# TheSandvichMaker/BUAS-Pathtracer

Hardware: AMD Instinct MI355X
Metric: Mrays/s + samples/s/GPU at 1080p 256spp; 1/2/4/8-GPU scaling (higher is better)
Workload: dtype f32

## Files before the change

buas-pathtracer_amd/abi.py:

```python
import ctypes as C
import os

PKG_DIR = os.path.dirname(os.path.abspath(__file__))
LIB_PATH = os.path.join(PKG_DIR, "lib", "librt_mi355x.so")

RT_OK = 0
RT_ERROR_INVALID = 1
RT_ERROR_DEVICE = 2
RT_ERROR_OUT_OF_MEMORY = 3
RT_ERROR_CANCELLED = 4
RT_ERROR_NO_DEVICE = 5

RT_MATERIAL_MIRROR = 0x1
RT_MATERIAL_CHECKERS = 0x2
RT_MATERIAL_EMISSIVE = 0x4

RT_PRIMITIVE_NONE, RT_PRIMITIVE_PLANE, RT_PRIMITIVE_SPHERE, RT_PRIMITIVE_BOX, RT_PRIMITIVE_MESH = range(5)
RT_SAMPLING_UNIFORM, RT_SAMPLING_OPTIMIZED_BLUE_NOISE, RT_SAMPLING_STRATIFIED = range(3)
RT_SPLAT_STREAM, RT_SPLAT_EXACT, RT_SPLAT_ATOMIC = range(3)
RT_SHARD_TILES, RT_SHARD_PASSES = range(2)
RT_SHADOW_LAUNCH_AUTO, RT_SHADOW_LAUNCH_SEPARATE, RT_SHADOW_LAUNCH_MERGED = range(3)
(RT_INTEGRATOR_ADVANCED, RT_INTEGRATOR_WHITTED, RT_INTEGRATOR_GROUND_TRUTH_RECURSIVE,
 RT_INTEGRATOR_GROUND_TRUTH_ITERATIVE, RT_INTEGRATOR_NORMALS, RT_INTEGRATOR_DISTANCES) = range(6)
RT_INTEGRATOR_COUNT = 6
# ... 184 lines not shown
                ("max_leaf_size", C.c_uint32)]


P = C.POINTER

ABI_FUNCTIONS = {
    "rt_abi_version": (C.c_int, []),
    "rt_last_error": (C.c_char_p, []),
    "rt_device_count": (C.c_int, [P(C.c_int)]),
    "rt_integrator_name": (C.c_char_p, [C.c_int]),
    "rt_find_integrator": (C.c_int, [C.c_char_p]),
    "rt_integrator_supported": (C.c_int, [C.c_int]),
    "rt_scene_set_recursive_integrators": (C.c_int, [C.c_void_p, C.c_int]),
    "rt_scene_integrator_supported": (C.c_int, [C.c_void_p, C.c_int]),
    "rt_scene_set_ambient_light": (C.c_int, [C.c_void_p, P(V3)]),
    "rt_scene_upload": (C.c_int, [P(SceneDesc), C.c_int, P(C.c_void_p)]),
    "rt_scene_free": (C.c_int, [C.c_void_p]),
    "rt_render": (C.c_int, [C.c_void_p, P(Camera), P(Settings), P(FilterCache), P(TileSet), C.c_uint32,
                            P(AccumulationBuffer), P(Stats)]),
    "rt_render_device": (C.c_int, [C.c_void_p, P(Camera), P(Settings), P(FilterCache), P(TileSet), C.c_uint32,
                                   C.c_uint32, C.c_uint32, C.c_uint32, C.c_void_p, C.c_void_p, P(Stats)]),
    "rt_trace_samples": (C.c_int, [C.c_void_p, P(Camera), P(Settings), C.c_uint32, C.c_uint32, C.c_uint32,
                                   C.c_uint32, C.c_uint32, C.c_uint32, C.c_uint32, P(C.c_uint32), P(C.c_uint32),
                                   P(C.c_float), P(Stats)]),
    "rt_debug_intersect": (C.c_int, [C.c_void_p, C.c_uint32, P(RayQuery), C.c_int, P(HitRecord)]),
    "rt_debug_mesh_bvh4": (C.c_int, [P(BvhNode), C.c_uint32, P(C.c_float), C.c_uint32, P(C.c_uint32),
                                     P(C.c_uint32)]),
    "rt_debug_top_sequences": (C.c_int, [P(BvhNode), C.c_uint32, C.c_uint32, P(C.c_float), C.c_uint32,
                                         P(C.c_uint32)]),
    "rt_debug_claim_slots": (C.c_int, [P(C.c_uint32), C.c_uint32, C.c_uint32, C.c_uint32, P(C.c_uint32)]),
    "rt_debug_rank_slots": (C.c_int, [P(C.c_uint32), C.c_uint32, C.c_uint32, C.c_uint32, P(C.c_uint32)]),
    "rt_scene_ramp_stats": (C.c_int, [C.c_void_p, P(C.c_uint64), P(C.c_uint64)]),
    "rt_debug_verify_rcp": (C.c_int, [C.c_int, P(C.c_uint64), P(C.c_uint32)]),
    "rt_set_profiling": (C.c_int, [C.c_int]),
    "rt_set_profiling_stages": (C.c_int, [C.c_uint32]),
    "rt_set_path_pool": (C.c_int, [C.c_uint32]),
    "rt_set_splat_mode": (C.c_int, [C.c_int]),
    "rt_set_shard_mode": (C.c_int, [C.c_int]),
    "rt_set_env_sampling": (C.c_int, [C.c_int]),
    "rt_build_bvh": (C.c_int, [C.c_int, C.c_uint32, P(V3), P(V3), C.c_int, P(BvhNode), P(C.c_uint32), P(C.c_uint32)]),
    "rt_build_bvh_last_error": (C.c_char_p, []),
    "rt_render_picture": (C.c_int, [C.c_void_p, P(Camera), P(Settings), P(FilterCache), P(TileSet), C.c_uint32,
                                    C.c_uint32, C.c_uint32, P(PostSettings), P(C.c_uint32), P(Stats)]),
    "rt_cancel": (C.c_int, [C.c_void_p]),
    "rt_scene_default_config": (C.c_int, [P(SceneConfig)]),
    "rt_scene_get_config": (C.c_int, [C.c_void_p, P(SceneConfig)]),
    "rt_scene_set_config": (C.c_int, [C.c_void_p, P(SceneConfig)]),
    "rt_scene_stack_depth": (C.c_int, [C.c_void_p, P(C.c_uint32), P(C.c_uint32)]),
    "rt_postprocess_device": (C.c_int, [C.c_int, C.c_void_p, C.c_uint32, C.c_uint32, P(PostSettings), C.c_uint32,
                                        C.c_void_p, C.c_void_p]),
    "rt_postprocess": (C.c_int, [C.c_int, P(AccumulationBuffer), P(PostSettings), C.c_uint32, P(C.c_uint32)]),
    "rt_denoise_default_params": (C.c_int, [P(DenoiseParams)]),
    "rt_denoise_workspace_bytes": (C.c_size_t, [C.c_uint32, C.c_uint32]),
    "rt_denoise_device": (C.c_int, [C.c_int, C.c_void_p, C.c_void_p, C.c_void_p, C.c_uint32, C.c_uint32,
                                    P(DenoiseParams), C.c_void_p, C.c_void_p, C.c_void_p]),
    "rt_denoise": (C.c_int, [C.c_int, P(AccumulationBuffer), P(C.c_float), P(C.c_float), P(DenoiseParams),
                             P(C.c_float)]),
    "rt_render_picture_denoised": (C.c_int, [C.c_void_p, P(Camera), P(Settings), P(FilterCache), P(TileSet),
                                             C.c_uint32, C.c_uint32, C.c_uint32, P(PostSettings), P(DenoiseParams),
                                             C.c_uint32, P(C.c_uint32), P(Stats)]),
    "rt_render_feature_device": (C.c_int, [C.c_void_p, P(Camera), P(Settings), P(FilterCache), P(TileSet), C.c_uint32,
                                           C.c_uint32, C.c_uint32, C.c_uint32, C.c_int, C.c_void_p, C.c_void_p,
                                           P(Stats)]),
    "rt_render_feature": (C.c_int, [C.c_void_p, P(Camera), P(Settings), P(FilterCache), P(TileSet), C.c_uint32,
                                    C.c_int, P(AccumulationBuffer), P(Stats)]),
    "rt_render_features_device": (C.c_int, [C.c_void_p, P(Camera), P(Settings), P(FilterCache), P(TileSet), C.c_uint32,
# ... 121 lines not shown
```

buas-pathtracer_amd/csrc/rt_dmath.h:

```cpp
#pragma once
#include <hip/hip_runtime.h>
#include <stdint.h>
#include "../../include/rt_abi.h"

#ifdef RT_DMATH_HOST_TEST
#define RT_D inline
#else
#define RT_D __device__ __forceinline__
#endif

namespace rtd {

constexpr float PI_32 = 3.14159265359f;
constexpr float TAU_32 = 6.28318530717f;
constexpr float EPSILON = 0.001f;
constexpr float FLT_MAX_ = 3.402823466e+38F;

struct V3 { float x, y, z; };
struct V2 { float x, y; };

RT_D V3 v3(float x, float y, float z) { return {x, y, z}; }
RT_D V3 v3s(float s) { return {s, s, s}; }
RT_D V3 add(V3 a, V3 b) { return {a.x + b.x, a.y + b.y, a.z + b.z}; }
RT_D V3 sub(V3 a, V3 b) { return {a.x - b.x, a.y - b.y, a.z - b.z}; }
RT_D V3 mul(V3 a, V3 b) { return {a.x * b.x, a.y * b.y, a.z * b.z}; }
RT_D V3 divv(V3 a, V3 b) { return {a.x / b.x, a.y / b.y, a.z / b.z}; }
RT_D V3 muls(V3 a, float s) { return {a.x * s, a.y * s, a.z * s}; }
RT_D V3 smul(float s, V3 a) { return {s * a.x, s * a.y, s * a.z}; }
RT_D V3 divs(V3 a, float s) { return {a.x / s, a.y / s, a.z / s}; }
RT_D V3 sdiv(float s, V3 a) { return {s / a.x, s / a.y, s / a.z}; }
RT_D V3 neg(V3 a) { return {-a.x, -a.y, -a.z}; }
RT_D float rcp_cr(float x) {
#ifndef RT_DMATH_HOST_TEST
    const float a = __builtin_fabsf(x);
    if (a >= 0x1p-125f && a <= 0x1p125f) {
        const float r = __builtin_amdgcn_rcpf(x);
        return __builtin_fmaf(__builtin_fmaf(-x, r, 1.0f), r, r);
    }
#endif
    return 1.0f / x;
}
RT_D V3 rcp3(V3 a) { return {rcp_cr(a.x), rcp_cr(a.y), rcp_cr(a.z)}; }
RT_D float dot(V3 a, V3 b) { return a.x*b.x + a.y*b.y + a.z*b.z; }
RT_D V3 cross(V3 a, V3 b) { return {a.y*b.z - a.z*b.y, a.z*b.x - a.x*b.z, a.x*b.y - a.y*b.x}; }
RT_D float length_sq(V3 a) { return dot(a, a); }
RT_D float mn(float a, float b) { return a < b ? a : b; }
RT_D float mx(float a, float b) { return a > b ? a : b; }
RT_D float clampf_(float n, float a, float b) { return mx(a, mn(b, n)); }
RT_D float max3(V3 a) { return mx(a.x, mx(a.y, a.z)); }
RT_D V3 vabs(V3 a) { return {fabsf(a.x), fabsf(a.y), fabsf(a.z)}; }
RT_D V3 normalize(V3 a) { float r = rcp_cr(__builtin_sqrtf(dot(a, a))); return muls(a, r); }
RT_D V3 noz(V3 a) {
    V3 r = {0.0f, 0.0f, 0.0f};
    float lsq = length_sq(a);
    if ((lsq > 0.0001f) && (lsq < __builtin_inff())) r = divs(a, __builtin_sqrtf(lsq));
    return r;
}
RT_D float lerpf_(float a, float b, float t) { return a*(1.0f - t) + b*t; }
RT_D V3 lerp3(V3 a, V3 b, float t) { return add(muls(a, 1.0f - t), muls(b, t)); }
RT_D V3 reflect(V3 v, V3 n) { return sub(v, muls(n, 2.0f*dot(v, n))); }
RT_D float sign_of(float x) { return x < 0.0f ? -1.0f : 1.0f; }
RT_D float copy_sign(float v, float s) {
    return __uint_as_float((__float_as_uint(s) & 0x80000000u) | (__float_as_uint(v) & 0x7FFFFFFFu));
}
RT_D float comp(V3 a, int i) { return i == 0 ? a.x : (i == 1 ? a.y : a.z); }

struct M34 { float e[3][4]; };

RT_D V3 xform(const M34& a, V3 p, float pw) {
    return {p.x*a.e[0][0] + p.y*a.e[0][1] + p.z*a.e[0][2] + pw*a.e[0][3],
            p.x*a.e[1][0] + p.y*a.e[1][1] + p.z*a.e[1][2] + pw*a.e[1][3],
            p.x*a.e[2][0] + p.y*a.e[2][1] + p.z*a.e[2][2] + pw*a.e[2][3]};
}
RT_D V3 xform_normal(const M34& a, V3 n) {
    return {n.x*a.e[0][0] + n.y*a.e[0][1] + n.z*a.e[2][0],
// ... 195 lines not shown
```

buas-pathtracer_amd/csrc/rt_kernels.hip:

```cpp
#include <hip/hip_runtime.h>
#include <stdint.h>
#include <string.h>
#include <stdio.h>
#include <string>
#include <vector>
#include <chrono>
#include <algorithm>
#include <type_traits>
#include <cmath>
#include <mutex>
#include <cerrno>

#include "rt_dmath.h"

using namespace rtd;

#define HIP_OK(x) do { hipError_t e_ = (x); if (e_ != hipSuccess) { set_error(std::string(#x) + ": " + hipGetErrorString(e_)); return RT_ERROR_DEVICE; } } while (0)

namespace {
thread_local std::string g_error;
void set_error(const std::string& s) { g_error = s; }
uint32_t g_profiling = 0;
uint32_t g_pool_override = 0;
int g_splat_mode = RT_SPLAT_STREAM;
// ... 42 lines not shown
    uint32_t sky_w, sky_h;
    const float4* env_tab;
    uint32_t env_n, env_tx, env_tw, env_th;
    V3 top_sky, bot_sky;
    const uint8_t* strata;
    const uint8_t* bluenoise;
    const float4* blob;
    uint32_t blob_q;
    uint32_t off[7];
};
enum { BLOB_MATERIALS, BLOB_PRIMS, BLOB_PLANES, BLOB_INV, BLOB_FWD, BLOB_LIGHTS, BLOB_MESHES, BLOB_COUNT };
constexpr uint32_t LDS_SCENE_Q = 2048;
extern __shared__ float4 lds_scene[];

template <bool IN_LDS = false>
RT_D DevScene scene_in_lds(const DevScene& sc, float4* lds) {
    if (!IN_LDS && !sc.blob_q) return sc;
    for (uint32_t i = threadIdx.x; i < sc.blob_q; i += blockDim.x) lds[i] = sc.blob[i];
    __syncthreads();
    DevScene s = sc;
    const char* b = reinterpret_cast<const char*>(lds);
    s.materials = reinterpret_cast<const rt_material*>(b + sc.off[BLOB_MATERIALS]);
    s.prims = reinterpret_cast<const rt_primitive*>(b + sc.off[BLOB_PRIMS]);
    s.planes = reinterpret_cast<const rt_primitive*>(b + sc.off[BLOB_PLANES]);
    s.inv = reinterpret_cast<const M34*>(b + sc.off[BLOB_INV]);
    s.fwd = reinterpret_cast<const M34*>(b + sc.off[BLOB_FWD]);
    s.lights = reinterpret_cast<const uint32_t*>(b + sc.off[BLOB_LIGHTS]);
    s.meshes = reinterpret_cast<const DevMesh*>(b + sc.off[BLOB_MESHES]);
    return s;
}

struct Ray { V3 o, d, inv_d; uint32_t neg; float max_t; uint32_t zero; };

RT_D Ray make_ray(V3 o, V3 d, float far_clip) {
    Ray r;
    r.o = o; r.d = d;
    r.inv_d = rcp3(d);
    r.neg = (d.x < 0.0f ? 1u : 0u) | (d.y < 0.0f ? 2u : 0u) | (d.z < 0.0f ? 4u : 0u);
    r.zero = (d.x == 0.0f ? 1u : 0u) | (d.y == 0.0f ? 2u : 0u) | (d.z == 0.0f ? 4u : 0u);
    r.max_t = far_clip;
    return r;
}

RT_D bool ray_plane(const Ray& ray, V3 n, float d, float& t) {
    float denom = dot(n, ray.d);
    if (denom < -EPSILON) {
        float tt = (d - dot(n, ray.o)) / denom;
        if ((tt >= EPSILON) && (tt < t)) { t = tt; return true; }
    }
    return false;
}
RT_D bool ray_sphere(const Ray& ray, float r, float& t) {
    V3 o = ray.o;
    float rsq = r*r;
    float b = dot(ray.d, o);
    float c = dot(o, o) - rsq;
    float discr = (b*b - c);
    if (discr >= 0) {
        float root = __builtin_sqrtf(discr);
        float tn = -b - root;
        float tf = -b + root;
        float tt = (tn >= 0.0f ? tn : tf);
        if ((tt >= EPSILON) && (t > tt)) { t = tt; return true; }
    }
    return false;
}
RT_D bool ray_box(const Ray& ray, V3 br, float& t) {
    V3 m = ray.inv_d;
    V3 n = mul(m, ray.o);
    V3 k = mul(vabs(m), br);
    V3 t1 = sub(neg(n), k);
    V3 t2 = add(neg(n), k);
// ... 207 lines not shown
        return r;
    }
    const float4* seq = sc.top_seq;
    uint32_t list = 0, n = 0, next = 0;
    bool full = false;
    const uint32_t len = sc.top_seq_len;
    const bool plain = plain_ray(o, d);
    for (uint32_t i = 0; i < len; ++i) {
        const f32x8 e = ld_uniform_v<f32x8>(seq + 2*i);
        const float4 a = q4_of(e, 0), b = q4_of(e, 1);
        const uint32_t info = __float_as_uint(b.z), skip = __float_as_uint(b.w);
        bool pass = false;
        if (next == i) {
            float tn;
            pass = bv_static(wr, {a.x, a.y, a.z}, {a.w, b.x, b.y}, tn) && tn < r.t;
            next = pass ? ((info >> 31) ? skip : i + 1) : skip;
        }
        if (!(info >> 31) || __ballot(pass) == 0ull) continue;
        const uint32_t first = info & 0xFFFFFFu, end = first + ((info >> 24) & 127u);
        for (uint32_t j = first; j < end; ++j) {
            const float4* q = sc.leaf_rec + (size_t)j*LEAF_REC_Q;
            const f32x16 qa = ld_uniform_v<f32x16>(q);
            const float4 q3 = q4_of(qa, 3);
            const uint32_t pi = __float_as_uint(q3.x), tword = __float_as_uint(q3.y), type = tword & 0xFFu;
            if (!pass || pi == ignored) continue;
            const float4 q0 = q4_of(qa, 0), q1 = q4_of(qa, 1), q2 = q4_of(qa, 2);
            V3 io, id;
            object_ray(q0, q1, q2, tword & LEAF_TRANSLATE, plain, o, d, io, id);
            bool hit = false;
            if (type == RT_PRIMITIVE_SPHERE) {
                Ray ir; ir.o = io; ir.d = id;
                hit = ray_sphere(ir, q3.z, r.t);
            } else {
                const Ray ir = make_ray(io, id, 0.0f);
                if (type == RT_PRIMITIVE_MESH) {
                    const f32x8 qb = ld_uniform_v<f32x8>(q + 4);
                    const float4 q4 = q4_of(qb, 0), q5 = q4_of(qb, 1);
                    float tm;
                    n += 1u << 8;
                    if (bv_static(ir, {q4.y, q4.z, q4.w}, {q5.x, q5.y, q5.z}, tm) && tm < r.t) {
                        const uint32_t k = n & 0xFFu;
                        if (k < sc.mlist_max) list |= j << (6*k);
                        else full = true;
                        ++n;
                    }
                    continue;
                }
                if (type == RT_PRIMITIVE_BOX) hit = ray_box(ir, {q3.z, q3.w, ld_uniform(q + 4).x}, r.t);
            }
            if (hit) {
                r.code = pi;
                if (occ) { r.occluded = true; pass = false; next = 0xFFFFFFFFu; }
            }
        }
    }
    r.calls = n >> 8;
    if (r.occluded) return r;
    n &= 0xFFu;
    r.bvh = n > 0;
    r.mlist = full ? MLIST_FULL : (list | (n << 24));
    return r;
}

template <bool LST>
struct StepField {
    static constexpr uint32_t B = LST ? 8 : 6, M = (1u << B) - 1u;
    static constexpr uint32_t ENTRY = 1u, NODE = 1u << B, LEAF = 1u << 2*B, TRIS = 1u << 3*B,
// ... 127 lines not shown
    }

    template <bool SH>
    RT_D bool pop(const Stack& st, const rt_bvh_node* nodes, int base) {
        while (sp > base) {
            const uint2 e = st.template get<SH>(--sp);
            if (REF && e.x == REF_MARKER) {
                if (__uint_as_float(e.y) < t) { rp[0] += 2u; rp[1] += 1u; }
                continue;
            }
            if (__uint_as_float(e.y) < t) {
                unpack_node(nodes, e.x, cur_lf, cur_cnt, cur_ax);
                has_cur = true;
                return true;
            }
        }
        return false;
    }

    template <bool SH, bool FIN>
    RT_D void push_children4(const Stack& st, const float4* F, const float4* mid = nullptr) {
        const Ray r = cur_ray();
        const uint32_t meta = __float_as_uint(F[7].x), nb = cflags & 7u;
        const uint32_t g = (nb >> (meta & 3u)) & 1u;
        const uint32_t fa = (nb >> ((meta >> 2) & 3u)) & 1u;
        const uint32_t fb = (nb >> ((meta >> 4) & 3u)) & 1u;
        const uint32_t rec[4] = {__float_as_uint(F[6].x), __float_as_uint(F[6].y), __float_as_uint(F[6].z), __float_as_uint(F[6].w)};
        float tn[4];
        bool h[4];
        h[0] = bv_static<FIN>(r, {F[0].x, F[1].x, F[2].x}, {F[3].x, F[4].x, F[5].x}, tn[0]) && rec[0] != EMPTY4;
        h[1] = bv_static<FIN>(r, {F[0].y, F[1].y, F[2].y}, {F[3].y, F[4].y, F[5].y}, tn[1]) && rec[1] != EMPTY4;
        h[2] = bv_static<FIN>(r, {F[0].z, F[1].z, F[2].z}, {F[3].z, F[4].z, F[5].z}, tn[2]) && rec[2] != EMPTY4;
        h[3] = bv_static<FIN>(r, {F[0].w, F[1].w, F[2].w}, {F[3].w, F[4].w, F[5].w}, tn[3]) && rec[3] != EMPTY4;
        const uint32_t f1 = g ? fb : fa, f2 = g ? fa : fb;
        const uint32_t v[4] = {2u*g + f1, 2u*g + 1u - f1, 2u*(1u - g) + f2, 2u*(1u - g) + 1u - f2};
        bool far_marker = false;
        float far_tn = 0.0f;
        if (REF) {
            rp[0] += 2u; rp[1] += 1u;
            const V3 pc[2] = {{mid[0].x, mid[0].y, mid[0].z}, {mid[1].z, mid[1].w, mid[2].x}};
            const V3 rr[2] = {{mid[0].w, mid[1].x, mid[1].y}, {mid[2].y, mid[2].z, mid[2].w}};
#pragma unroll
            for (uint32_t c = 0; c < 2; ++c) {
                if ((c == 0 ? rec[1] : rec[3]) == EMPTY4) continue;
                float tc;
                const bool hc = bv_static<FIN>(r, pc[c], rr[c], tc);
                if (c == g) { if (hc && tc < t) { rp[0] += 2u; rp[1] += 1u; } }
                else if (hc) { far_marker = true; far_tn = tc; }
            }
        }
#pragma unroll
        for (int k = 3; k >= 0; --k) {
            const uint32_t i = v[k];
            const bool hi = i == 0 ? h[0] : i == 1 ? h[1] : i == 2 ? h[2] : h[3];
            const uint32_t ri = i == 0 ? rec[0] : i == 1 ? rec[1] : i == 2 ? rec[2] : rec[3];
            const float ti = i == 0 ? tn[0] : i == 1 ? tn[1] : i == 2 ? tn[2] : tn[3];
            if (hi) push<SH>(st, ri, ti);
            if (REF && k == 2 && far_marker) push<SH>(st, REF_MARKER, far_tn);
        }
    }

    static constexpr int PUSH_MAX = REF ? 5 : 4;
    using SF = StepField<LST>;
    uint32_t acc = 0;
    RT_D bool step(const DevScene& sc, const Stack& st) {
        if (__ballot(sp > SL - PUSH_MAX || !(cflags & 64u)) == 0ull) return step_impl<true, true>(sc, st);
// ... 1074 lines not shown
                }
                ro = add(I, smul(EPSILON, nd)); rd = nd;
                thr = mul(thr, lerp3(v3s(1.0f), rv3(mt.albedo), mt.metallic));
            } else if (mt.is_participating_medium) {
                if (inside) {
                    if (at > 0) --at;
                } else if (at < 63) {
                    ++at;
                    pool.mstack[(size_t)at*pool.n + slot] = (uint16_t)mt_id;
                }
                V3 fd = add(smul(eta, rd), muls(N, (eta*cos_i - cos_t)));
                ro = add(I, muls(fd, EPSILON)); rd = fd;
            } else {
                is_spec = 0;
                V3 albedo = evaluate_material(mt, I);
                V3 brdf = smul(1.0f / PI_32, albedo);
                if (st.next_event_estimation && (sc.light_count > 0 || ENV)) {
                    float lps = sample_1d(sc, ss, rng, S_LightSelection, bounce);
                    const float q = sc.light_count > 0 ? 0.5f : 1.0f;
                    const bool pick_env = ENV && lps < q;
                    if (ENV) lps = pick_env ? lps / q : (lps - q) / (1.0f - q);
                    float lrp = 0.0f;
                    uint32_t lid = pick_env ? 0u : pick_random_light(sc, st, lps, I, lrp);
                    if (ENV) lrp = lrp*(1.0f - q);
                    V2 s2 = sample_2d(sc, ss, rng, S_DirectLighting, bounce);
                    if (pick_env) {
                        V3 Lv = env_direction(sc, lps, s2);
                        float ndl = dot(N, Lv);
                        if (ndl > 0.0f) {
                            uint32_t tile;
                            V3 Le = sky_env(sc, Lv, tile);
                            float pe = env_pdf(sc, tile, Lv);
                            if (pe > 0.0f) {
                                float bpdf = (st.importance_sample_diffuse ? ndl / PI_32 : 1.0f / (2.0f*PI_32));
                                float pdf = st.use_mis ? q*pe + bpdf : q*pe;
                                sh_c = mul(mul(muls(thr, ndl / pdf), brdf), Le);
                                sh_o = add(I, muls(Lv, EPSILON));
                                sh_d = Lv;
                                sh_t = FLT_MAX_;
                                sh_light = 0;
                                cast_shadow = true;
                            }
                        }
                    } else {
                        const rt_primitive light = sc.prims[lid];
                        const M34 lf = load_m34(&sc.fwd[light.transform_index]);
                        V3 towards = normalize(sub(translation(lf), I));
                        if (light.type == RT_PRIMITIVE_SPHERE) {
                            float rad = light.p[0];
                            V3 Nl = map_to_hemisphere(neg(towards), s2);
                            V3 pw = xform(lf, muls(Nl, rad), 1.0f);
                            V3 Lv = sub(pw, I);
                            float dsq = length_sq(Lv);
                            float dist = __builtin_sqrtf(dsq);
                            Lv = divs(Lv, dist);
                            float A = 2.0f*PI_32*rad*rad;
                            float ndl = dot(N, Lv);
                            float nndl = -dot(Nl, Lv);
                            if (ndl > 0.0f && nndl > 0.0f) {
                                float sa = (nndl * A) / dsq;
                                float pdf;
                                if (st.use_mis) {
                                    float lpdf = rcp_cr(sa);
                                    float bpdf = (st.importance_sample_diffuse ? ndl / PI_32 : 1.0f / (2.0f*PI_32));
                                    pdf = lpdf + bpdf;
                                } else {
                                    pdf = rcp_cr(sa);
                                }
                                pdf *= lrp;
                                sh_c = mul(mul(muls(thr, dot(N, Lv) / pdf), brdf),
                                           rv3(sc.materials[light.material_id].emission_color));
                                sh_o = add(I, muls(Lv, EPSILON));
                                sh_d = Lv;
                                sh_t = dist - 2*EPSILON;
                                sh_light = lid;
                                cast_shadow = true;
                            }
                        }
                    }
                }
                V2 s2 = sample_2d(sc, ss, rng, S_IndirectLighting, bounce);
                V3 R;
                if (st.importance_sample_diffuse) {
                    R = map_to_cosine_weighted_hemisphere(N, s2);
                    thr = muls(thr, PI_32);
                } else {
                    R = map_to_hemisphere(N, s2);
                    thr = muls(thr, 2.0f*PI_32*dot(N, R));
                }
                thr = mul(thr, brdf);
                ro = add(I, muls(N, EPSILON)); rd = R;
            }
            if (st.russian_roulette && !is_spec) {
                float p = clampf_(max3(thr), 0.1f, 0.9f);
                float e = sample_1d(sc, ss, rng, S_Roulette, bounce);
                if (e > p) done = true;
                else thr = muls(thr, rcp_cr(p));
            }
        }
        if (!done) {
            if (st.importance_sample_diffuse) prev_pdf = dot(N, rd) / PI_32;
            ++bounce;
            if (bounce >= st.max_bounce_count) done = true;
        }
    } else {
        if (ENV) {
            uint32_t tile;
            V3 Le = sky_env(sc, rd, tile);
            if (!is_spec) {
                float wgt = 0.0f;
                if (st.use_mis) {
                    const float q = sc.light_count > 0 ? 0.5f : 1.0f;
                    float pe = env_pdf(sc, tile, rd);
                    float bpdf = (st.importance_sample_diffuse ? prev_pdf : 1.0f / (2.0f*PI_32));
                    float den = q*pe + bpdf;
                    wgt = den > 0.0f ? bpdf / den : 0.0f;
                }
                Le = smul(wgt, Le);
            }
            total = add(total, mul(thr, Le));
        } else {
            total = add(total, mul(thr, sample_sky(sc, rd)));
        }
        done = true;
    }
    return done;
}

template <int INTEG>
RT_D bool shade_bounce_gt(const DevScene& sc, const rt_settings& st, const Hit& h, V3& ro, V3& rd, V3& thr,
                          V3& total, uint32_t& bounce, Rng& rng) {
    constexpr bool FIRST_HIT = INTEG == RT_INTEGRATOR_NORMALS || INTEG == RT_INTEGRATOR_DISTANCES;
    if (h.code == RT_HIT_MISS) {
        if (FIRST_HIT) total = sample_sky(sc, rd);
// ... 647 lines not shown
                        ro = add(I, muls(nd, EPSILON)); rd = nd;
                    } else {
                        const V3 brdf = muls(evaluate_material(m, I), 1.0f / PI_32);
                        const V3 R = map_to_hemisphere(N, V2{r1, r2});
                        fs.put(level, 0, brdf, __uint_as_float(RF_DIFFUSE));
                        fs.put(level, 1, v3s(0.0f), mx(0.0f, dot(N, R)));
                        ro = add(I, muls(N, EPSILON)); rd = R;
                    }
                    ++level;
                }
            }
        }
        if (WHITTED) {
            V3 ill = {0, 0, 0};
            const uint32_t nlights = __ballot(lit) ? sc.light_count : 0u;
            for (uint32_t li = 0; li < nlights; ++li) {
                bool cast_shadow = false;
                V3 sh_o = {0, 0, 0}, sh_d = {0, 0, 0}, sh_c = {0, 0, 0};
                float sh_t = 0.0f;
                uint32_t sh_light = 0;
                if (lit) {
                    const uint32_t lid = sc.lights[li];
                    const rt_primitive light = sc.prims[lid];
                    const V2 s2 = sample_2d(sc, ss, rng, S_DirectLighting, 0);
                    if (light.type == RT_PRIMITIVE_SPHERE) {
                        const M34 lf = load_m34(&sc.fwd[light.transform_index]);
                        const V3 towards = normalize(sub(translation(lf), I));
                        const float rad = light.p[0];
                        const V3 Nl = map_to_hemisphere(neg(towards), s2);
                        const V3 pw = xform(lf, muls(Nl, rad), 1.0f);
                        V3 Lv = sub(pw, I);
                        const float dsq = length_sq(Lv);
                        const float dist = __builtin_sqrtf(dsq);
                        Lv = divs(Lv, dist);
                        const float A = 2.0f*PI_32*rad*rad;
                        const float ndl = dot(N, Lv);
                        const float nndl = -dot(Nl, Lv);
                        if (ndl > 0.0f && nndl > 0.0f) {
                            sh_o = add(I, muls(Lv, EPSILON));
                            sh_d = Lv;
                            sh_t = dist - 2*EPSILON;
                            sh_light = lid;
                            sh_c = divs(smul(nndl*A*ndl, rv3(sc.materials[light.material_id].emission_color)), dsq);
                            cast_shadow = true;
                        }
                    }
                }
                Prologue spro = {};
                if (cast_shadow) spro = ray_prologue(sc, sh_o, sh_d, sh_t, true, sh_light);
                n_calls[1] += cast_shadow ? spro.calls : 0u;
                Traversal<true, LST, STACK_LDS, REF> tr;
                bool tracing = cast_shadow && !spro.occluded && spro.bvh;
                n_traced_sh += tracing ? 1u : 0u;
                if (tracing) {
                    tr.init_rec(sc, stk, sh_o, sh_d, spro.inv_d, sh_t, sh_light, spro.mlist);
                    tracing = tr.mode != TM_DONE;
                }
                for (int k = 1; __ballot(tracing); ++k) {
                    if (tracing && !tr.step(sc, stk)) tracing = false;
                    if (k % StepField<LST>::H == 0) tally[1].flush(tr.acc);
                }
                tally[1].flush(tr.acc);
                if (REF) tally[1].flush_ref(tr.rc);
                if (cast_shadow && !spro.occluded && (!spro.bvh || !tr.occluded)) ill = add(ill, sh_c);
                n_shadow += cast_shadow ? 1u : 0u;
            }
            if (lit) {
// ... 493 lines not shown
RT_D float post_clamp(float n, float a, float b) { return mx(a, mn(b, n)); }
RT_D float sigmoidal_contrast(float x, float contrast, float midpoint) {
    float curve;
    if (x < midpoint) {
        float scale = (1.0f / midpoint)*x;
        curve = midpoint*(scale*scale);
    } else {
        float y = (1.0f / (1.0f - midpoint));
        float scale = y - y*x;
        curve = 1.0f - (1.0f - midpoint)*(scale*scale);
    }
    return lerpf_(x, curve, contrast);
}
RT_D float remap_tpdf(float x) {
    float orig = 2.0f*x - 1.0f;
    x = orig*(1.0f / __builtin_sqrtf(fabsf(orig)));
    x = mx(-1.0f, x);
    x = x - sign_of(x);
    return x;
}
__global__ void __launch_bounds__(256) k_verify_rcp(uint32_t base, unsigned long long* out) {
    const uint32_t t = blockIdx.x*256 + threadIdx.x, stride = gridDim.x*256;
    for (uint32_t i = 0; i < 16; ++i) {
        const uint32_t bits = base + t + i*stride;
        const float x = __uint_as_float(bits);
        const float a = rcp_cr(x), b = 1.0f / x;
        if (__float_as_uint(a) != __float_as_uint(b) && !(a != a && b != b)) {
            atomicAdd(out, 1ull);
            atomicMin(out + 1, (unsigned long long)bits);
        }
    }
}

__global__ void __launch_bounds__(256) k_post(const float4* px, uint32_t w, uint32_t h, rt_post_settings post,
                                              const uint8_t* noise, uint32_t* out) {
    const uint32_t x = blockIdx.x*64 + (threadIdx.x & 63), y = blockIdx.y*4 + (threadIdx.x >> 6);
    if (x >= w || y >= h) return;
    const size_t i = (size_t)y*w + x;
    const float4 s = px[i];
    V3 c = {0.0f, 0.0f, 0.0f};
    if ((s.x != s.x) || (s.y != s.y) || (s.z != s.z) || (s.w != s.w)) {
        c = {0.0f, 255.0f, 255.0f};
    } else if (s.w > 0.001f) {
        c = {s.x / s.w, s.y / s.w, s.z / s.w};
        c = {mx(c.x, 0.0f), mx(c.y, 0.0f), mx(c.z, 0.0f)};
        if (post.exposure != 0.0f) c = smul(d_powf(2.0f, post.exposure), c);
        if (post.tonemapping) c = {1.0f - d_expf(-c.x), 1.0f - d_expf(-c.y), 1.0f - d_expf(-c.z)};
        if (post.srgb_transform) {
            const float g = 1.0f / 2.23333f;
            c = {d_powf(c.x, g), d_powf(c.y, g), d_powf(c.z, g)};
        }
        if (post.contrast != 0.0f)
            c = {sigmoidal_contrast(c.x, post.contrast, post.midpoint), sigmoidal_contrast(c.y, post.contrast, post.midpoint),
                 sigmoidal_contrast(c.z, post.contrast, post.midpoint)};
        c = smul(255.0f, c);
        const uint8_t* d = noise + 3*((size_t)(y & 255u)*256 + (x & 255u));
        c.x = c.x + (0.5f + remap_tpdf((1.0f / 255.0f)*(float)d[0]));
        c.y = c.y + (0.5f + remap_tpdf((1.0f / 255.0f)*(float)d[1]));
        c.z = c.z + (0.5f + remap_tpdf((1.0f / 255.0f)*(float)d[2]));
    } else if (s.w < -0.01f) {
        c = {-255.0f*s.w, 0.0f, -255.0f*s.w};
    }
    const uint32_t r = (uint8_t)post_clamp(c.x, 0.0f, 255.0f);
    const uint32_t g = (uint8_t)post_clamp(c.y, 0.0f, 255.0f);
    const uint32_t b = (uint8_t)post_clamp(c.z, 0.0f, 255.0f);
    out[i] = (255u << 24) | (r << 16) | (g << 8) | b;
// ... 1201 lines not shown
        auto within = [](const rt_bvh_node* n, size_t count) {
            for (size_t i = 0; i < count; ++i) {
                const float c[3] = {n[i].bv_p.x, n[i].bv_p.y, n[i].bv_p.z}, r[3] = {n[i].bv_r.x, n[i].bv_r.y, n[i].bv_r.z};
                for (int k = 0; k < 3; ++k)
                    if (!(std::fabs(c[k]) + std::fabs(r[k]) <= 1099511627776.0f)) return false;
            }
            return true;
        };
        ds.finite_boxes = (within(d->bvh_nodes, d->bvh_node_count) && within(mnodes.data(), mnodes.size())) ? 1u : 0u;
    }
    if (top_depth + mesh_depth + 2 > STACK_DEPTH) {
        char msg[224];
        snprintf(msg, sizeof(msg), "rt_scene_upload: BVH too deep for the device's BVH4 traversal stack: needs %u entries "
                 "(top level %u + mesh BVH4 %u + 2), %d available (the device's bound, not the reference's BVH2 stack)",
                 top_depth + mesh_depth + 2, top_depth, mesh_depth, STACK_DEPTH);
        set_error(msg);
        return fail(RT_ERROR_INVALID);
    }
    s->bvh_depth = top_depth + mesh_depth;
    s->bvh_depth_ref = top_depth + std::max(mesh_depth, mesh_depth_ref);
    if (s->cfg.traversal_ref && s->bvh_depth_ref + 2 > STACK_DEPTH) {
        set_error("rt_scene_upload: traversal_ref needs more than the 64-entry traversal stack for this BVH");
        return fail(RT_ERROR_INVALID);
    }
    {
        auto u2f = [](uint32_t u) { float f; memcpy(&f, &u, 4); return f; };
        std::vector<float4> rec((size_t)d->bvh_index_count*LEAF_REC_Q, make_float4(0, 0, 0, 0));
        for (uint32_t j = 0; j < d->bvh_index_count; ++j) {
            const uint32_t pi = d->bvh_indices[j];
            const rt_primitive& p = d->primitives[pi];
            float4* q = rec.data() + (size_t)j*LEAF_REC_Q;
            const M34& iv = inv[p.transform_index];
            for (int r = 0; r < 3; ++r) q[r] = make_float4(iv.e[r][0], iv.e[r][1], iv.e[r][2], iv.e[r][3]);
            if (p.type == RT_PRIMITIVE_MESH) {
                const rt_mesh& M = d->meshes[p.mesh_index];
                rt_bvh_node rn = {};
                if (M.node_count) rn = M.nodes[0];
                const uint32_t root = root4[p.mesh_index];
                q[3] = make_float4(u2f(pi), u2f(p.type), u2f(meshes[p.mesh_index].node_offset), u2f(meshes[p.mesh_index].tri_offset));
                q[4] = make_float4(u2f(root), rn.bv_p.x, rn.bv_p.y, rn.bv_p.z);
                if (M.node_count) q[5] = make_float4(rn.bv_r.x, rn.bv_r.y, rn.bv_r.z, 1.0f);
                else q[5] = make_float4(-1.0f, -1.0f, -1.0f, 0.0f);
            } else {
                bool translate = std::isfinite(iv.e[0][3]) && std::isfinite(iv.e[1][3]) && std::isfinite(iv.e[2][3]);
                for (int r = 0; r < 3; ++r)
                    for (int c = 0; c < 3; ++c) translate = translate && iv.e[r][c] == (r == c ? 1.0f : 0.0f);
                q[3] = make_float4(u2f(pi), u2f(p.type | (translate ? LEAF_TRANSLATE : 0u)), p.p[0], p.p[1]);
                q[4] = make_float4(p.p[2], 0.0f, 0.0f, 0.0f);
            }
        }
        rec.resize(rec.size() + FETCH_Q, make_float4(0, 0, 0, 0));
        if ((err = upload(s, rec.data(), rec.size(), &ds.leaf_rec))) return fail(err);
    }
    if ((err = upload(s, meshes.data(), meshes.size(), &ds.meshes))) return fail(err);
    tris.resize(tris.size() + FETCH_Q, make_float4(0, 0, 0, 0));
    if ((err = upload(s, tris.data(), tris.size(), &ds.tris))) return fail(err);
    if ((err = upload(s, orig.data(), orig.size(), &ds.tri_orig))) return fail(err);
    if ((err = upload(s, normals.data(), normals.size(), &ds.normals))) return fail(err);
    mnodes.resize(mnodes.size() + (FETCH_Q*16 + 31)/32, rt_bvh_node{});
    if ((err = upload(s, mnodes.data(), mnodes.size(), &ds.mnodes_src))) return fail(err);
    {
        std::vector<rt_bvh_node> tl(mnodes.size());
        for (uint32_t m = 0; m < d->mesh_count; ++m) {
            const uint32_t off = meshes[m].node_offset, n = d->meshes[m].node_count;
            std::vector<rt_bvh_node> one = traversal_layout(mnodes.data() + off, n);
            std::copy(one.begin(), one.end(), tl.begin() + off);
        }
        if ((err = upload(s, tl.data(), tl.size(), &ds.mnodes))) return fail(err);
    }
    ds.mnodes4 = nullptr;
    {
        const uint32_t n4 = (uint32_t)(mnodes4.size() / 8);
        bool bad = false;
        for (uint32_t m = 0; m < d->mesh_count; ++m)
            bad |= root4[m] < (1u << 28) && root4[m] >= n4 && d->meshes[m].node_count && !d->meshes[m].nodes[0].count;
        for (size_t k = 0; k < n4 && !bad; ++k)
            for (int j = 0; j < 4; ++j) {
                uint32_t r;
                memcpy(&r, &(&mnodes4[8*k + 6].x)[j], 4);
                bad |= r != EMPTY4 && r < (1u << 28) && r >= n4;
// ... 777 lines not shown
    return RT_OK;
}

int rt_debug_top_sequences(const rt_bvh_node* nodes, uint32_t node_count, uint32_t index_count,
                           float* out, uint32_t out_cap_entries, uint32_t* out_len) {
    if (!nodes || !out_len) { set_error("null argument"); return RT_ERROR_INVALID; }
    uint32_t len = 0;
    std::vector<float4> q = top_sequences(nodes, node_count, index_count, len);
    *out_len = len;
    if (q.empty()) { set_error("top level too large for the prologue"); return RT_ERROR_INVALID; }
    if (out && out_cap_entries >= 8*len) memcpy(out, q.data(), q.size()*sizeof(float4));
    return (out && out_cap_entries < 8*len) ? RT_ERROR_INVALID : RT_OK;
}

int rt_debug_verify_rcp(int device, uint64_t* out_mismatches, uint32_t* out_first_bits) {
    if (!out_mismatches || !out_first_bits) { set_error("null argument"); return RT_ERROR_INVALID; }
    int err = bind_device(device);
    if (err) return err;
    unsigned long long* d = nullptr;
    HIP_OK(hipMalloc(&d, 2*sizeof(unsigned long long)));
    const unsigned long long init[2] = {0ull, 0xFFFFFFFFull};
    HIP_OK(hipMemcpy(d, init, sizeof(init), hipMemcpyHostToDevice));
    for (uint32_t chunk = 0; chunk < 16; ++chunk)
        k_verify_rcp<<<(1u << 28) / (256*16), 256>>>(chunk << 28, d);
    HIP_OK(hipGetLastError());
    unsigned long long h[2];
    HIP_OK(hipMemcpy(h, d, sizeof(h), hipMemcpyDeviceToHost));
    (void)hipFree(d);
    *out_mismatches = h[0];
    *out_first_bits = (uint32_t)h[1];
    return RT_OK;
}

int rt_debug_intersect(rt_scene* s, uint32_t count, const rt_ray_query* rays, int occlusion, rt_hit_record* out) {
    if (!s || !rays || !out) { set_error("null argument"); return RT_ERROR_INVALID; }
    if (!count) return RT_OK;
    HIP_OK(hipSetDevice(s->device));
    rt_ray_query* d_r = nullptr; rt_hit_record* d_o = nullptr;
    HIP_OK(hipMalloc(&d_r, sizeof(rt_ray_query)*count));
    HIP_OK(hipMalloc(&d_o, sizeof(rt_hit_record)*count));
    HIP_OK(hipMemcpy(d_r, rays, sizeof(rt_ray_query)*count, hipMemcpyHostToDevice));
    uint2* d_sp = nullptr;
    const uint32_t dgrid = (count + 127) / 128;
    HIP_OK(hipMalloc(&d_sp, sizeof(uint2)*(size_t)(STACK_DEPTH - STACK_LDS)*dgrid*128));
    if (occlusion) k_debug_intersect<true><<<dgrid, 128>>>(s->ds, d_r, d_o, count, d_sp);
    else k_debug_intersect<false><<<dgrid, 128>>>(s->ds, d_r, d_o, count, d_sp);
    HIP_OK(hipGetLastError());
    HIP_OK(hipDeviceSynchronize());
    (void)hipFree(d_sp);
    HIP_OK(hipMemcpy(out, d_o, sizeof(rt_hit_record)*count, hipMemcpyDeviceToHost));
    (void)hipFree(d_r); (void)hipFree(d_o);
    return RT_OK;
}

}

#include "rt_internal.h"
void rt_internal_set_error(const char* message) { set_error(message); }
int rt_internal_bind_device(int device) { return bind_device(device); }
int rt_internal_scene_device(const rt_scene* scene) { return scene->device; }
int rt_internal_scene_cancelled(const rt_scene* scene) { return scene->cancel; }
```

include/rt_abi.h:

```cpp
#ifndef RT_ABI_H
#define RT_ABI_H

#include <stdint.h>
#include <stddef.h>

#ifdef __cplusplus
extern "C" {
#endif

#define RT_ABI_VERSION 8

enum rt_status {
    RT_OK                 = 0,
    RT_ERROR_INVALID      = 1,
    RT_ERROR_DEVICE       = 2,
    RT_ERROR_OUT_OF_MEMORY= 3,
    RT_ERROR_CANCELLED    = 4,
    RT_ERROR_NO_DEVICE    = 5,
};

typedef struct rt_v3 { float x, y, z; } rt_v3;
typedef struct rt_m4x4 { float e[4][4]; } rt_m4x4;
typedef struct rt_m4x4inv { rt_m4x4 forward, inverse; } rt_m4x4inv;

// ... 211 lines not shown
              const rt_filter_cache* filter, const rt_tile_set* tiles,
              uint32_t total_frame_index, rt_accumulation_buffer* accum, rt_stats* stats);

int rt_render_device(rt_scene* scene, const rt_camera* camera, const rt_settings* settings,
                     const rt_filter_cache* filter, const rt_tile_set* tiles,
                     uint32_t total_frame_index, uint32_t w, uint32_t h, uint32_t frame_count,
                     float* d_pixels, void* hip_stream, rt_stats* stats);

int rt_render_picture(rt_scene* scene, const rt_camera* camera, const rt_settings* settings,
                      const rt_filter_cache* filter, const rt_tile_set* tiles, uint32_t total_frame_index,
                      uint32_t w, uint32_t h, const rt_post_settings* post, uint32_t* out_bgra, rt_stats* stats);

int rt_trace_samples(rt_scene* scene, const rt_camera* camera, const rt_settings* settings,
                     uint32_t w, uint32_t h, uint32_t tile_w, uint32_t tile_h,
                     uint32_t frame_count, uint32_t total_frame_index,
                     uint32_t count, const uint32_t* pixel_xy, const uint32_t* sample_offset,
                     float* out_rgbjj, rt_stats* stats);

int rt_debug_intersect(rt_scene* scene, uint32_t count, const rt_ray_query* rays,
                       int occlusion, rt_hit_record* out);

int rt_debug_mesh_bvh4(const rt_bvh_node* nodes, uint32_t node_count, float* out, uint32_t out_cap_nodes,
                       uint32_t* out_nodes, uint32_t* out_root_record);
int rt_debug_top_sequences(const rt_bvh_node* nodes, uint32_t node_count, uint32_t index_count,
                           float* out, uint32_t out_cap_entries, uint32_t* out_len);

int rt_debug_claim_slots(const uint32_t* free_w, uint32_t nwaves, uint32_t first_claim, uint32_t count,
                         uint32_t* out_slots);
int rt_debug_rank_slots(const uint32_t* free_w, uint32_t nwaves, uint32_t first_rank, uint32_t count,
                        uint32_t* out_slots);
int rt_scene_ramp_stats(const rt_scene* scene, uint64_t* out_iterations, uint64_t* out_paths);

int rt_debug_verify_rcp(int device, uint64_t* out_mismatches, uint32_t* out_first_bits);

int rt_postprocess_device(int device, const float* d_pixels, uint32_t w, uint32_t h,
                          const rt_post_settings* post, uint32_t total_frame_index,
                          uint32_t* d_bgra, void* hip_stream);

int rt_postprocess(int device, const rt_accumulation_buffer* accum, const rt_post_settings* post,
                   uint32_t total_frame_index, uint32_t* out_bgra);

typedef struct rt_denoise_params {
    int32_t iterations;
    float   sigma_color;
    float   sigma_guide[2];
    float   firefly_clamp;
    int32_t reserved[3];
} rt_denoise_params;
int    rt_denoise_default_params(rt_denoise_params* out);
size_t rt_denoise_workspace_bytes(uint32_t w, uint32_t h);
int rt_denoise_device(int device, const float* d_beauty, const float* d_guide0, const float* d_guide1,
                      uint32_t w, uint32_t h, const rt_denoise_params* p, void* d_workspace,
                      float* d_out, void* hip_stream);
int rt_denoise(int device, const rt_accumulation_buffer* beauty, const float* guide0, const float* guide1,
               const rt_denoise_params* p, float* out_pixels);
int rt_render_picture_denoised(rt_scene* scene, const rt_camera* camera, const rt_settings* settings,
                               const rt_filter_cache* filter, const rt_tile_set* tiles, uint32_t total_frame_index,
                               uint32_t w, uint32_t h, const rt_post_settings* post, const rt_denoise_params* p,
                               uint32_t guide_spp, uint32_t* out_bgra, rt_stats* stats);

enum rt_feature { RT_FEATURE_NORMAL = 0, RT_FEATURE_DISTANCE = 1, RT_FEATURE_ALBEDO = 2, RT_FEATURE_COUNT = 3 };
int rt_render_feature_device(rt_scene* scene, const rt_camera* camera, const rt_settings* settings,
                             const rt_filter_cache* filter, const rt_tile_set* tiles, uint32_t total_frame_index,
                             uint32_t w, uint32_t h, uint32_t frame_count, int feature, float* d_pixels,
                             void* hip_stream, rt_stats* stats);
int rt_render_feature(rt_scene* scene, const rt_camera* camera, const rt_settings* settings,
// ... 165 lines not shown
```

Baseline: 14400.

## Replace IEEE divides with exact reciprocal-FMA sequences and reuse world inv_d for translated instances

Replaces divisions by PI and by the light distance with reciprocal-multiply plus FMA correction sequences meant to give bit-identical results, and adds device verification entry points for both. Mesh instances whose transform is a pure translation now carry the LEAF_TRANSLATE flag, so when a whole wave qualifies the world ray's inverse direction is reused instead of recomputing three reciprocals. The BVH4 child push in the non-reference path is rewritten as branch-free slot arithmetic. These trim ALU work in shading and traversal, at the cost of extra range checks and code size.

Result: faster. 14780 (median of 6 runs) (+2.6%).

```diff
diff --git a/buas-pathtracer_amd/abi.py b/buas-pathtracer_amd/abi.py
--- a/buas-pathtracer_amd/abi.py
+++ b/buas-pathtracer_amd/abi.py
@@ -240,6 +240,8 @@
     "rt_debug_rank_slots": (C.c_int, [P(C.c_uint32), C.c_uint32, C.c_uint32, C.c_uint32, P(C.c_uint32)]),
     "rt_scene_ramp_stats": (C.c_int, [C.c_void_p, P(C.c_uint64), P(C.c_uint64)]),
     "rt_debug_verify_rcp": (C.c_int, [C.c_int, P(C.c_uint64), P(C.c_uint32)]),
+    "rt_debug_verify_div_pi": (C.c_int, [C.c_int, P(C.c_uint64), P(C.c_uint32)]),
+    "rt_debug_verify_div3": (C.c_int, [C.c_int, C.c_uint32, P(C.c_float), P(C.c_uint64), P(C.c_uint32)]),
     "rt_set_profiling": (C.c_int, [C.c_int]),
     "rt_set_profiling_stages": (C.c_int, [C.c_uint32]),
     "rt_set_path_pool": (C.c_int, [C.c_uint32]),
diff --git a/buas-pathtracer_amd/csrc/rt_dmath.h b/buas-pathtracer_amd/csrc/rt_dmath.h
--- a/buas-pathtracer_amd/csrc/rt_dmath.h
+++ b/buas-pathtracer_amd/csrc/rt_dmath.h
@@ -41,6 +41,36 @@
     return 1.0f / x;
 }
 RT_D V3 rcp3(V3 a) { return {rcp_cr(a.x), rcp_cr(a.y), rcp_cr(a.z)}; }
+struct ByPi {
+    static constexpr float D = PI_32, C = 0x1.45f306p-2f;
+};
+static_assert(ByPi::C == 1.0f / ByPi::D, "ByPi::C is the rounded reciprocal of PI_32");
+template <class K>
+RT_D float div_const(float x) {
+    const float a = __builtin_fabsf(x);
+    if (a >= 0x1p-100f && a <= FLT_MAX_) {
+        const float q0 = x * K::C;
+        return __builtin_fmaf(__builtin_fmaf(-K::D, q0, x), K::C, q0);
+    }
+    return x / K::D;
+}
+RT_D float div_pi(float x) { return div_const<ByPi>(x); }
+constexpr float DIV3_LO = 0x1p-46f, DIV3_HI = 0x1p46f;
+RT_D bool div3_in_range(float x) { const float a = __builtin_fabsf(x); return a >= DIV3_LO && a <= DIV3_HI; }
+RT_D V3 div3_by(V3 n, float d) {
+#ifndef RT_DMATH_HOST_TEST
+    if (div3_in_range(d) && div3_in_range(n.x) && div3_in_range(n.y) && div3_in_range(n.z)) {
+        const float r0 = __builtin_amdgcn_rcpf(d);
+        const float r = __builtin_fmaf(__builtin_fmaf(-d, r0, 1.0f), r0, r0);
+        V3 q = {n.x * r, n.y * r, n.z * r};
+        q = {__builtin_fmaf(__builtin_fmaf(-d, q.x, n.x), r, q.x), __builtin_fmaf(__builtin_fmaf(-d, q.y, n.y), r, q.y),
+             __builtin_fmaf(__builtin_fmaf(-d, q.z, n.z), r, q.z)};
+        return {__builtin_fmaf(__builtin_fmaf(-d, q.x, n.x), r, q.x), __builtin_fmaf(__builtin_fmaf(-d, q.y, n.y), r, q.y),
+                __builtin_fmaf(__builtin_fmaf(-d, q.z, n.z), r, q.z)};
+    }
+#endif
+    return {n.x / d, n.y / d, n.z / d};
+}
 RT_D float dot(V3 a, V3 b) { return a.x*b.x + a.y*b.y + a.z*b.z; }
 RT_D V3 cross(V3 a, V3 b) { return {a.y*b.z - a.z*b.y, a.z*b.x - a.x*b.z, a.x*b.y - a.y*b.x}; }
 RT_D float length_sq(V3 a) { return dot(a, a); }
diff --git a/buas-pathtracer_amd/csrc/rt_kernels.hip b/buas-pathtracer_amd/csrc/rt_kernels.hip
--- a/buas-pathtracer_amd/csrc/rt_kernels.hip
+++ b/buas-pathtracer_amd/csrc/rt_kernels.hip
@@ -98,12 +98,17 @@
 
 struct Ray { V3 o, d, inv_d; uint32_t neg; float max_t; uint32_t zero; };
 
-RT_D Ray make_ray(V3 o, V3 d, float far_clip) {
+RT_D Ray make_ray_dir(V3 o, V3 d) {
     Ray r;
     r.o = o; r.d = d;
-    r.inv_d = rcp3(d);
     r.neg = (d.x < 0.0f ? 1u : 0u) | (d.y < 0.0f ? 2u : 0u) | (d.z < 0.0f ? 4u : 0u);
     r.zero = (d.x == 0.0f ? 1u : 0u) | (d.y == 0.0f ? 2u : 0u) | (d.z == 0.0f ? 4u : 0u);
+    r.max_t = 0.0f;
+    return r;
+}
+RT_D Ray make_ray(V3 o, V3 d, float far_clip) {
+    Ray r = make_ray_dir(o, d);
+    r.inv_d = rcp3(d);
     r.max_t = far_clip;
     return r;
 }
@@ -377,7 +382,9 @@
                 Ray ir; ir.o = io; ir.d = id;
                 hit = ray_sphere(ir, q3.z, r.t);
             } else {
-                const Ray ir = make_ray(io, id, 0.0f);
+                Ray ir = make_ray_dir(io, id);
+                if (__ballot(!((tword & LEAF_TRANSLATE) && plain)) == 0ull) ir.inv_d = wr.inv_d;
+                else ir.inv_d = rcp3(id);
                 if (type == RT_PRIMITIVE_MESH) {
                     const f32x8 qb = ld_uniform_v<f32x8>(q + 4);
                     const float4 q4 = q4_of(qb, 0), q5 = q4_of(qb, 1);
@@ -571,6 +578,23 @@
         h[1] = bv_static<FIN>(r, {F[0].y, F[1].y, F[2].y}, {F[3].y, F[4].y, F[5].y}, tn[1]) && rec[1] != EMPTY4;
         h[2] = bv_static<FIN>(r, {F[0].z, F[1].z, F[2].z}, {F[3].z, F[4].z, F[5].z}, tn[2]) && rec[2] != EMPTY4;
         h[3] = bv_static<FIN>(r, {F[0].w, F[1].w, F[2].w}, {F[3].w, F[4].w, F[5].w}, tn[3]) && rec[3] != EMPTY4;
+        if (!REF) {
+            uint32_t b0 = h[0] ? 1u : 0u, b1 = h[1] ? 1u : 0u, b2 = h[2] ? 1u : 0u, b3 = h[3] ? 1u : 0u;
+#ifdef __HIP_DEVICE_COMPILE__
+            asm volatile("" : "+v"(b0), "+v"(b1), "+v"(b2), "+v"(b3));
+#endif
+            const uint32_t nl = b0 + b1, nr = b2 + b3;
+            const uint32_t ol = g ? 0u : nr, orr = g ? nl : 0u;
+            const int l0 = sp + (int)(ol + (fa ? 0u : b1)), l1 = sp + (int)(ol + (fa ? b0 : 0u));
+            const int l2 = sp + (int)(orr + (fb ? 0u : b3)), l3 = sp + (int)(orr + (fb ? b2 : 0u));
+            if (b0 && (SH || l0 < STACK_DEPTH)) st.template put<SH>(l0, rec[0], tn[0]);
+            if (b1 && (SH || l1 < STACK_DEPTH)) st.template put<SH>(l1, rec[1], tn[1]);
+            if (b2 && (SH || l2 < STACK_DEPTH)) st.template put<SH>(l2, rec[2], tn[2]);
+            if (b3 && (SH || l3 < STACK_DEPTH)) st.template put<SH>(l3, rec[3], tn[3]);
+            sp += (int)(nl + nr);
+            if (!SH && sp > STACK_DEPTH) sp = STACK_DEPTH;
+            return;
+        }
         const uint32_t f1 = g ? fb : fa, f2 = g ? fa : fb;
         const uint32_t v[4] = {2u*g + f1, 2u*g + 1u - f1, 2u*(1u - g) + f2, 2u*(1u - g) + 1u - f2};
         bool far_marker = false;
@@ -1711,7 +1735,7 @@
                             V3 Le = sky_env(sc, Lv, tile);
                             float pe = env_pdf(sc, tile, Lv);
                             if (pe > 0.0f) {
-                                float bpdf = (st.importance_sample_diffuse ? ndl / PI_32 : 1.0f / (2.0f*PI_32));
+                                float bpdf = (st.importance_sample_diffuse ? div_pi(ndl) : 1.0f / (2.0f*PI_32));
                                 float pdf = st.use_mis ? q*pe + bpdf : q*pe;
                                 sh_c = mul(mul(muls(thr, ndl / pdf), brdf), Le);
                                 sh_o = add(I, muls(Lv, EPSILON));
@@ -1732,7 +1756,7 @@
                             V3 Lv = sub(pw, I);
                             float dsq = length_sq(Lv);
                             float dist = __builtin_sqrtf(dsq);
-                            Lv = divs(Lv, dist);
+                            Lv = div3_by(Lv, dist);
                             float A = 2.0f*PI_32*rad*rad;
                             float ndl = dot(N, Lv);
                             float nndl = -dot(Nl, Lv);
@@ -1741,7 +1765,7 @@
                                 float pdf;
                                 if (st.use_mis) {
                                     float lpdf = rcp_cr(sa);
-                                    float bpdf = (st.importance_sample_diffuse ? ndl / PI_32 : 1.0f / (2.0f*PI_32));
+                                    float bpdf = (st.importance_sample_diffuse ? div_pi(ndl) : 1.0f / (2.0f*PI_32));
                                     pdf = lpdf + bpdf;
                                 } else {
                                     pdf = rcp_cr(sa);
@@ -1778,7 +1802,7 @@
             }
         }
         if (!done) {
-            if (st.importance_sample_diffuse) prev_pdf = dot(N, rd) / PI_32;
+            if (st.importance_sample_diffuse) prev_pdf = div_pi(dot(N, rd));
             ++bounce;
             if (bounce >= st.max_bounce_count) done = true;
         }
@@ -2492,7 +2516,7 @@
                         V3 Lv = sub(pw, I);
                         const float dsq = length_sq(Lv);
                         const float dist = __builtin_sqrtf(dsq);
-                        Lv = divs(Lv, dist);
+                        Lv = div3_by(Lv, dist);
                         const float A = 2.0f*PI_32*rad*rad;
                         const float ndl = dot(N, Lv);
                         const float nndl = -dot(Nl, Lv);
@@ -3052,6 +3076,31 @@
     }
 }
 
+__global__ void __launch_bounds__(256) k_verify_div_pi(uint32_t base, unsigned long long* out) {
+    const uint32_t t = blockIdx.x*256 + threadIdx.x, stride = gridDim.x*256;
+    for (uint32_t i = 0; i < 16; ++i) {
+        const uint32_t bits = base + t + i*stride;
+        const float x = __uint_as_float(bits);
+        const float a = div_const<ByPi>(x), b = x / PI_32;
+        if (__float_as_uint(a) != __float_as_uint(b) && !(a != a && b != b)) {
+            atomicAdd(out, 1ull);
+            atomicMin(out + 1, (unsigned long long)bits);
+        }
+    }
+}
+__global__ void __launch_bounds__(256) k_verify_div3(const float4* sets, uint32_t count, unsigned long long* out) {
+    const uint32_t i = blockIdx.x*256 + threadIdx.x;
+    if (i >= count) return;
+    const float4 s = sets[i];
+    const V3 a = div3_by({s.x, s.y, s.z}, s.w);
+    const V3 b = {s.x / s.w, s.y / s.w, s.z / s.w};
+    auto differ = [](float p, float q) { return __float_as_uint(p) != __float_as_uint(q) && !(p != p && q != q); };
+    if (differ(a.x, b.x) || differ(a.y, b.y) || differ(a.z, b.z)) {
+        atomicAdd(out, 1ull);
+        atomicMin(out + 1, (unsigned long long)i);
+    }
+}
+
 __global__ void __launch_bounds__(256) k_post(const float4* px, uint32_t w, uint32_t h, rt_post_settings post,
                                               const uint8_t* noise, uint32_t* out) {
     const uint32_t x = blockIdx.x*64 + (threadIdx.x & 63), y = blockIdx.y*4 + (threadIdx.x >> 6);
@@ -4319,20 +4368,21 @@
             float4* q = rec.data() + (size_t)j*LEAF_REC_Q;
             const M34& iv = inv[p.transform_index];
             for (int r = 0; r < 3; ++r) q[r] = make_float4(iv.e[r][0], iv.e[r][1], iv.e[r][2], iv.e[r][3]);
+            bool translate = std::isfinite(iv.e[0][3]) && std::isfinite(iv.e[1][3]) && std::isfinite(iv.e[2][3]);
+            for (int r = 0; r < 3; ++r)
+                for (int c = 0; c < 3; ++c) translate = translate && iv.e[r][c] == (r == c ? 1.0f : 0.0f);
+            const uint32_t tword = p.type | (translate ? LEAF_TRANSLATE : 0u);
             if (p.type == RT_PRIMITIVE_MESH) {
                 const rt_mesh& M = d->meshes[p.mesh_index];
                 rt_bvh_node rn = {};
                 if (M.node_count) rn = M.nodes[0];
                 const uint32_t root = root4[p.mesh_index];
-                q[3] = make_float4(u2f(pi), u2f(p.type), u2f(meshes[p.mesh_index].node_offset), u2f(meshes[p.mesh_index].tri_offset));
+                q[3] = make_float4(u2f(pi), u2f(tword), u2f(meshes[p.mesh_index].node_offset), u2f(meshes[p.mesh_index].tri_offset));
                 q[4] = make_float4(u2f(root), rn.bv_p.x, rn.bv_p.y, rn.bv_p.z);
                 if (M.node_count) q[5] = make_float4(rn.bv_r.x, rn.bv_r.y, rn.bv_r.z, 1.0f);
                 else q[5] = make_float4(-1.0f, -1.0f, -1.0f, 0.0f);
             } else {
-                bool translate = std::isfinite(iv.e[0][3]) && std::isfinite(iv.e[1][3]) && std::isfinite(iv.e[2][3]);
-                for (int r = 0; r < 3; ++r)
-                    for (int c = 0; c < 3; ++c) translate = translate && iv.e[r][c] == (r == c ? 1.0f : 0.0f);
-                q[3] = make_float4(u2f(pi), u2f(p.type | (translate ? LEAF_TRANSLATE : 0u)), p.p[0], p.p[1]);
+                q[3] = make_float4(u2f(pi), u2f(tword), p.p[0], p.p[1]);
                 q[4] = make_float4(p.p[2], 0.0f, 0.0f, 0.0f);
             }
         }
@@ -5176,6 +5226,49 @@
     return RT_OK;
 }
 
+int rt_debug_verify_div_pi(int device, uint64_t* out_mismatches, uint32_t* out_first_bits) {
+    if (!out_mismatches || !out_first_bits) { set_error("null argument"); return RT_ERROR_INVALID; }
+    int err = bind_device(device);
+    if (err) return err;
+    unsigned long long* d = nullptr;
+    HIP_OK(hipMalloc(&d, 2*sizeof(unsigned long long)));
+    const unsigned long long init[2] = {0ull, 0xFFFFFFFFull};
+    HIP_OK(hipMemcpy(d, init, sizeof(init), hipMemcpyHostToDevice));
+    for (uint32_t chunk = 0; chunk < 16; ++chunk)
+        k_verify_div_pi<<<(1u << 28) / (256*16), 256>>>(chunk << 28, d);
+    HIP_OK(hipGetLastError());
+    unsigned long long h[2];
+    HIP_OK(hipMemcpy(h, d, sizeof(h), hipMemcpyDeviceToHost));
+    (void)hipFree(d);
+    *out_mismatches = h[0];
+    *out_first_bits = (uint32_t)h[1];
+    return RT_OK;
+}
+
+int rt_debug_verify_div3(int device, uint32_t count, const float* sets, uint64_t* out_mismatches, uint32_t* out_first_index) {
+    if (!sets || !out_mismatches || !out_first_index) { set_error("null argument"); return RT_ERROR_INVALID; }
+    *out_mismatches = 0; *out_first_index = 0xFFFFFFFFu;
+    if (!count) return RT_OK;
+    int err = bind_device(device);
+    if (err) return err;
+    float4* d_s = nullptr;
+    unsigned long long* d = nullptr;
+    HIP_OK(hipMalloc(&d_s, sizeof(float4)*(size_t)count));
+    HIP_OK(hipMalloc(&d, 2*sizeof(unsigned long long)));
+    const unsigned long long init[2] = {0ull, 0xFFFFFFFFull};
+    HIP_OK(hipMemcpy(d, init, sizeof(init), hipMemcpyHostToDevice));
+    HIP_OK(hipMemcpy(d_s, sets, sizeof(float4)*(size_t)count, hipMemcpyHostToDevice));
+    k_verify_div3<<<(count + 255) / 256, 256>>>(d_s, count, d);
+    HIP_OK(hipGetLastError());
+    unsigned long long h[2];
+    HIP_OK(hipMemcpy(h, d, sizeof(h), hipMemcpyDeviceToHost));
+    (void)hipFree(d_s);
+    (void)hipFree(d);
+    *out_mismatches = h[0];
+    *out_first_index = (uint32_t)h[1];
+    return RT_OK;
+}
+
 int rt_debug_intersect(rt_scene* s, uint32_t count, const rt_ray_query* rays, int occlusion, rt_hit_record* out) {
     if (!s || !rays || !out) { set_error("null argument"); return RT_ERROR_INVALID; }
     if (!count) return RT_OK;
diff --git a/include/rt_abi.h b/include/rt_abi.h
--- a/include/rt_abi.h
+++ b/include/rt_abi.h
@@ -267,6 +267,11 @@
 int rt_scene_ramp_stats(const rt_scene* scene, uint64_t* out_iterations, uint64_t* out_paths);
 
 int rt_debug_verify_rcp(int device, uint64_t* out_mismatches, uint32_t* out_first_bits);
+
+int rt_debug_verify_div_pi(int device, uint64_t* out_mismatches, uint32_t* out_first_bits);
+
+int rt_debug_verify_div3(int device, uint32_t count, const float* sets, uint64_t* out_mismatches,
+                         uint32_t* out_first_index);
 
 int rt_postprocess_device(int device, const float* d_pixels, uint32_t w, uint32_t h,
                           const rt_post_settings* post, uint32_t total_frame_index,
```
